# boqian333/E2ENet-Medical

Hardware: AMD Instinct MI355X
Metric: voxels/sec (train step fwd+bwd+update), 128^3 patch 32ch density=0.2 (higher is better)
Workload: dtype f32 (fp16x2 split products, f32 accumulate); 1 GPU; BraTS-shaped 4-modal 128^3 patches, shiftConvPP base 32, K=4, DSFF density 0.2, batch 2 per GPU, fwd+loss+bwd+clip+SGD+mask step, dense (parity) wgrad; parallelism=dp1

## Files before the change

### e2enet_medical_amd/_lib.py

```python
import ctypes as C
import os

_HERE = os.path.dirname(os.path.abspath(__file__))
LIB_PATH = os.environ.get("E2E_LIB_PATH") or os.path.join(_HERE, "csrc", "libe2e_hip.so")

KNOWN_ENV = frozenset({
    "E2E_CONV_MM", "E2E_MM_GRID", "E2E_MM_GEOM", "E2E_MM_PAIRQ", "E2E_CONV_DENSE", "E2E_CONV_SPARSE2", "E2E_CONV_PERSIST", "E2E_CONV_WGS",
    "E2E_CONV_KSPLIT", "E2E_WG_H2", "E2E_WG_BF3", "E2E_CT_BF3", "E2E_CT_H2",
    "E2E_CONV_DBG", "E2E_MM_STAMPS",
    "E2E_LIB_PATH", "E2E_STRICT_ENV", "E2E_DENSE_MIN_DENSITY", "E2E_MM_MIN_DENSITY", "E2E_WGRAD_STREAM", "E2E_LANES", "E2E_GRAPHS",
    "E2E_GRAPH_MAX_VOXELS", "E2E_PLAN_CACHE_GB", "E2E_SW_BLOCKING", "E2E_FORCE_DIST",
    "E2E_CPU_THREADS", "E2E_BENCH_DRY", "E2E_BENCH_DRY_FAIL_RANK", "E2E_BENCH_ALL_LAUNCHES",
})


def check_env(environ=None, strict=None):
    environ = os.environ if environ is None else environ
    unknown = sorted(k for k in environ if k.startswith("E2E_") and k not in KNOWN_ENV)
    if not unknown:
        return
    msg = ("unknown E2E_* environment variable(s) %s: not read by this build (known: %s)"
           % (", ".join(unknown), ", ".join(sorted(KNOWN_ENV))))
    if strict is None:
        strict = environ.get("E2E_STRICT_ENV") == "1"
# ... 70 lines not shown
    "e2e_conv133_sparse_eligible": (I, [I, I, I, I, I, I, I, I]),
    "e2e_conv133_sparse_wpk_floats": (LL, [I, I, I]),
    "e2e_conv133_sparse_plan": (I, [P, I, I, I, P, P, P, P, P, P]),
    "e2e_conv133_sparse_pack": (I, [P, I, LL, P]),
    "e2e_conv133_fwd_sparse": (I, [P, I, P, P, P, P, I, P, I, P, P, I, I, I, I, I, P]),
    "e2e_conv133_dgrad_sparse": (I, [P, P, P, P, I, P, P, P, I, I, I, I, I, I, I, P]),
    "e2e_conv133_fwd_dense": (I, [P, I, P, P, P, P, P, I, I, I, I, I, P, LL, P]),
    "e2e_conv133_mm_ws_bytes": (LL, [I, I, I, I, I, I, I, I, I]),
    "e2e_conv133_mm_pack": (I, [P, I, LL, P]),
    "e2e_conv133_input_ranges_ws_bytes": (LL, [I]),
    "e2e_conv133_input_ranges": (I, [P, I, P, P]),
    "e2e_absmax_word": (I, [P, LL, P, P]),
    "e2e_conv133_fwd_mm": (I, [P, I, P, P, P, P, P, P, I, I, I, I, I, P]),
    "e2e_conv133_dgrad_mm": (I, [P, P, P, P, P, I, I, I, I, I, I, P]),
    "e2e_conv133_dgrad_dense": (I, [P, P, P, P, I, I, I, I, I, I, P, LL, P]),
    "e2e_conv133_wgrad_ws_bytes": (LL, [I, I, I, I, I, I, I, I, I]),
    "e2e_conv133_wgrad": (I, [P, P, P, P, I, I, I, I, I, I, I, I, I, P, P, P]),
    "e2e_diag_split_gemm": (I, [P, P, P, I, I, P, P]),
    "e2e_diag_kernel_clock": (I, [I, P, P, I]),
    "e2e_in_stats_finalize": (I, [P, I, P, P, F, P, P, P, P, I, I, P]),
    "e2e_in_lrelu_bwd_ws_doubles": (LL, [I, I]),
    "e2e_in_lrelu_bwd": (I, [P, P, P, P, P, P, P, F, P, P, P, P, I, I, LL, P, I, P, P]),
    "e2e_convT_fwd": (I, [P, P, P, F, P, P, P, I, I, I, I, I, I, I, I, I, P, P, P]),
    "e2e_convT_dgrad": (I, [P, P, P, P, I, I, I, I, I, I, I, I, I, I, P, P, P, P]),
    "e2e_convT_wgrad_ws_bytes": (LL, [I, I, I, I, I, I, I, I, I]),
    "e2e_convT_wgrad": (I, [P, P, P, F, P, P, P, I, I, I, I, I, I, I, I, I, P, P, P, P]),
    "e2e_maxpool_fwd": (I, [P, P, P, F, P, I, I, I, I, I, I, I, I, P]),
    "e2e_maxpool_bwd_num_records": (I, [I, I, I, I, I, I]),
    "e2e_maxpool_bwd": (I, [P, P, P, F, P, P, I, I, I, I, I, I, I, I, I, P, P, P, P]),
    "e2e_head1x1_fwd": (I, [P, P, P, F, P, P, I, I, I, LL, P]),
    "e2e_head1x1_dgrad": (I, [P, P, P, I, I, I, I, LL, P]),
    "e2e_head1x1_wgrad_ws_bytes": (LL, [I, I, I, LL]),
    "e2e_head1x1_wgrad": (I, [P, P, P, F, P, P, P, I, I, I, LL, P]),
    "e2e_loss_ws_bytes": (LL, [I, I]),
    "e2e_dc_ce_reduce": (I, [P, P, P, I, I, LL, P]),
    "e2e_dc_ce_grad": (I, [P, P, P, F, I, F, P, P, I, I, LL, P]),
    "e2e_dc_ce_fold_batch": (I, [P, I, I, P]),
    "e2e_online_eval_counts": (I, [P, P, P, I, I, LL, P]),
    "e2e_dc_bce_reduce": (I, [P, P, P, P, I, I, LL, P]),
    "e2e_dc_bce_grad": (I, [P, P, P, P, F, I, F, P, P, I, I, LL, P]),
    "e2e_online_eval_regions": (I, [P, P, P, P, I, I, LL, P]),
    "e2e_seg_to_regions": (I, [P, P, P, I, I, LL, P]),
    "e2e_ds_target_gather": (I, [P, P, P, P, P, I, I, I, I, I, I, I, P]),
    "e2e_grad_sqnorm": (I, [P, I, P, P]),
    "e2e_sgd_clip_mask_step": (I, [P, I, P, F, F, F, F, I, I, P]),
    "e2e_apply_mask": (I, [P, I, P]),
    "e2e_dsff_kernel_l1": (I, [P, P, I, I, I, I, I, P]),
    "e2e_dsff_kth_value": (I, [P, I, I, P, P, P]),
    "e2e_dsff_death": (I, [P, P, P, I, P]),
    "e2e_dsff_grad_score": (I, [P, P, F, P, P, I, I, I, I, I, P]),
    "e2e_dsff_grow_above": (I, [P, P, P, I, I, I, P]),
    "e2e_dsff_expand": (I, [P, P, P, P, I, I, I, P]),
    "e2e_dsff_expand_quads": (I, [P, P, P, I, I, P]),
    "e2e_dsff_kmask_from_weights": (I, [P, P, I, I, I, P]),
    "e2e_flip3d": (I, [P, P, I, I, I, I, I, P]),
    "e2e_softmax_flip_acc": (I, [P, P, F, I, I, I, I, I, I, P]),
    "e2e_nonlin_flip_acc": (I, [P, P, F, I, I, I, I, I, I, I, P]),
    "e2e_sw_accumulate": (I, [P, P, P, P, I, I, I, I, I, I, I, I, I, I, P]),
    "e2e_sw_finalize_argmax": (I, [P, P, P, P, I, I, I, I, I, I, I, I, I, I, P]),
    "e2e_ensemble_accumulate": (I, [P, P, LL, I, I, P]),
    "e2e_export_argmax_u8": (I, [P, P, I, LL, I, I, I, LL, LL, LL, I, I, I, I, I, I, P, I, P]),
    "e2e_resample_linear": (I, [P, P, I, LL, I, I, I, LL, LL, LL, I, I, I, I, P]),
    "e2e_softmax_to_f16": (I, [P, P, I, LL, I, I, I, LL, LL, LL, P]),
    "e2e_merge_softmax_f16": (I, [P, I, I, I, I, I, P, I, I, I, I, I, I, P, I, P, P]),
    "e2e_aug_spatial": (I, [P, P, P, P, P, P, P, I, I, I, I, I, I, I, I, I, I, F, P]),
    "e2e_aug_bspline_prefilter_axis": (I, [P, P, I, I, I, I, I, P]),
# ... 26 lines not shown
    "e2e_pp_crop": (I, [P, P, P, P, P, I, I, I, I, I, I, I, I, I, I, I, F, P]),
    "e2e_pp_label_hist_bins": (I, []),
    "e2e_pp_label_hist": (I, [P, LL, P, I, P]),
    "e2e_pp_nan_to_zero": (I, [P, LL, P]),
    "e2e_pp_minmax_ws_bytes": (LL, [I, I, I, I, I]),
    "e2e_pp_minmax": (I, [P, P, P, I, LL, I, I, I, LL, LL, LL, I, P]),
    "e2e_pp_pad_edge": (I, [P, P, I, LL, I, I, I, LL, LL, LL, I, I, I, P]),
    "e2e_pp_resize_cubic": (I, [P, P, P, I, I, I, I, I, I, I, I, I, P]),
    "e2e_pp_resize_seg": (I, [P, P, I, LL, I, I, I, LL, LL, LL, I, I, I, I, P]),
    "e2e_pp_norm_ws_bytes": (LL, [I]),
    "e2e_pp_norm_stats": (I, [P, P, P, P, P, I, LL, P]),
    "e2e_pp_normalize": (I, [P, P, P, P, I, LL, P]),
    "e2e_pp_select_chunk": (I, []),
    "e2e_pp_select_max_classes": (I, []),
    "e2e_pp_select_ws_bytes": (LL, [LL, I]),
    "e2e_pp_select_count": (I, [P, LL, P, I, P, P, P]),
    "e2e_pp_select_coords": (I, [P, I, I, I, P, I, P, P, P, P, P, P]),
    "e2e_fingerprint_sample_chunk": (I, []),
    "e2e_fingerprint_sample_ws_bytes": (LL, [LL]),
    "e2e_fingerprint_sample_count": (I, [P, LL, P, P, P]),
    "e2e_fingerprint_sample_gather": (I, [P, P, I, LL, I, P, LL, P, P]),
    "e2e_fingerprint_stats_max_ranks": (I, []),
    "e2e_fingerprint_stats_ws_bytes": (LL, []),
    "e2e_fingerprint_stats": (I, [P, LL, P, I, P, P, P]),
    "e2e_loader_crop_max_batch": (I, []),
    "e2e_loader_crop": (I, [P, I, I, I, I, I, P, P, I, F, F, P]),
    "e2e_nifti_decode_f32": (I, [P, LL, I, I, I, C.c_double, C.c_double, P, P]),
    "e2e_nifti_decode_u8": (I, [P, LL, I, I, I, C.c_double, C.c_double, P, P, P]),
    "e2e_nifti_scan_grid_voxels": (LL, [I]),
    "e2e_nifti_scan": (I, [P, LL, I, I, I, C.c_double, C.c_double, P, P]),
}

_NO_STATUS = {"e2e_last_error", "e2e_abi_version", "e2e_last_kernel", "e2e_conv133_num_partials", "e2e_conv133_wgrad_ws_bytes", "e2e_conv133_dense_ws_bytes", "e2e_conv133_mm_ws_bytes", "e2e_conv133_sparse_eligible", "e2e_conv133_sparse_wpk_floats", "e2e_maxpool_bwd_num_records", "e2e_conv133_fwd_ws_bytes", "e2e_conv133_dgrad_ws_bytes",
              "e2e_convT_wgrad_ws_bytes", "e2e_conv133_input_ranges_ws_bytes", "e2e_in_lrelu_bwd_ws_doubles", "e2e_head1x1_wgrad_ws_bytes", "e2e_loss_ws_bytes", "e2e_aug_stats_ws_bytes",
              "e2e_surface_max_line", "e2e_surface_distances_ws_bytes", "e2e_cc_ws_bytes", "e2e_ct_ws_bytes", "e2e_pp_nonzero_ws_bytes", "e2e_pp_label_hist_bins",
              "e2e_pp_minmax_ws_bytes", "e2e_pp_norm_ws_bytes", "e2e_pp_select_chunk", "e2e_pp_select_max_classes", "e2e_pp_select_ws_bytes",
              "e2e_fingerprint_sample_chunk", "e2e_fingerprint_sample_ws_bytes", "e2e_fingerprint_stats_max_ranks",
              "e2e_fingerprint_stats_ws_bytes", "e2e_eval_census_max_slots", "e2e_eval_census_chunk", "e2e_eval_census_workgroups",
              "e2e_loader_crop_max_batch", "e2e_nifti_scan_grid_voxels"}


class E2EError(RuntimeError):
    pass


class _Lib:
    def __init__(self, path):
        if not os.path.exists(path):
            raise ImportError(
                "libe2e_hip.so not found at %s: build it with `python -c 'import __graft_entry__ as g; g.build()'` "
                "or `make -C e2enet_medical_amd/csrc`. There is no CPU fallback." % path)
        self._dll = C.CDLL(path)
        self.path = path
        for name, (res, args) in SIGNATURES.items():
            fn = getattr(self._dll, name)
            fn.restype = res
            fn.argtypes = args
            if name in _NO_STATUS:
                setattr(self, name[4:], fn)
            else:
                setattr(self, name[4:], self._checked(name, fn))

    def _checked(self, name, fn):
        last_error = self._dll.e2e_last_error

        def call(*a):
            rc = fn(*a)
            if rc != 0:
                raise E2EError("%s failed (%d): %s" % (name, rc, (last_error() or b"").decode()))
        call.__name__ = name
        return call


_lib = None


ABI_VERSION = 27


def lib() -> _Lib:
    global _lib
    if _lib is None:
        import torch
        check_env()
        handle = _Lib(LIB_PATH)
        got = handle.abi_version()
        if got != ABI_VERSION:
            raise ImportError("%s reports ABI version %d, this package needs %d: rebuild with `make -C %s`"
                              % (LIB_PATH, got, ABI_VERSION, os.path.dirname(LIB_PATH)))
        _lib = handle
    return _lib
```

### e2enet_medical_amd/csrc/api.hip

```cpp
#include "e2e_common.h"
#include <cstring>

namespace e2e {
static thread_local char g_err[512] = "";
void set_error(const char* fmt, ...) {
  va_list ap;
  va_start(ap, fmt);
  vsnprintf(g_err, sizeof(g_err), fmt, ap);
  va_end(ap);
}
static thread_local char g_kernel[160] = "";
void note_kernel(const char* fmt, ...) {
  va_list ap;
  va_start(ap, fmt);
  vsnprintf(g_kernel, sizeof(g_kernel), fmt, ap);
  va_end(ap);
}
}

extern "C" const char* e2e_last_error(void) { return e2e::g_err; }
extern "C" const char* e2e_last_kernel(void) { return e2e::g_kernel; }
extern "C" int e2e_abi_version(void) { return 27; }

extern "C" int e2e_diag_kernel_clock(int family, double* mhz, double* busy_ms, int reset) {
  E2E_REQUIRE(mhz != nullptr && (family == 0 || family == 1), "diag_kernel_clock: family 0 (conv133_mm) or 1 (conv133_wgrad v5)");
  if (hipDeviceSynchronize() != hipSuccess) return e2e::check_launch("diag_kernel_clock");
  unsigned long long v[2] = {0, 0};
  if (family == 0) e2e::mm_clock_read(v, reset != 0); else e2e::wgrad_clock_read(v, reset != 0);
  *mhz = v[1] ? 100.0 * (double)v[0] / (double)v[1] : 0.0;
  if (busy_ms) *busy_ms = (double)v[1] / 1e5;
  return e2e::check_launch("diag_kernel_clock");
}
```

### e2enet_medical_amd/csrc/pool_head.hip

```cpp
#include "e2e_common.h"

namespace {

__global__ __launch_bounds__(256) void maxpool_fwd_kernel(const float* __restrict__ x, const float* __restrict__ scale,
                                                          const float* __restrict__ shift, float slope,
                                                          float* __restrict__ y, int D, int H, int W, int kd, int kh, int kw,
                                                          int Do, int Ho, int Wo) {
  const int nc = blockIdx.y;
  const long long ospatial = (long long)Do * Ho * Wo;
  const long long oi = (long long)blockIdx.x * 256 + threadIdx.x;
  if (oi >= ospatial) return;
  const int wo = (int)(oi % Wo);
  const long long r = oi / Wo;
  const int ho = (int)(r % Ho), dq = (int)(r / Ho);
  float a = 1.f, b = 0.f, sl = 1.f;
  if (scale) { a = scale[nc]; b = shift[nc]; sl = slope; }
  const float* xp = x + (long long)nc * D * H * W;
  float m = -INFINITY;
  for (int i = 0; i < kd; ++i)
    for (int j = 0; j < kh; ++j)
      for (int k = 0; k < kw; ++k) {
        const float v = e2e::in_act(xp[((long long)(dq * kd + i) * H + (ho * kh + j)) * W + (wo * kw + k)], a, b, sl);
        m = (v > m || v != v) ? v : m;
      }
// ... 359 lines not shown
          const float z[4] = {e2e::in_act(q.x, a[i], b[i], sl[i]), e2e::in_act(q.y, a[i], b[i], sl[i]),
                              e2e::in_act(q.z, a[i], b[i], sl[i]), e2e::in_act(q.w, a[i], b[i], sl[i])};
#pragma unroll
          for (int k = 0; k < KB; ++k)
#pragma unroll
            for (int j = 0; j < 4; ++j) acc[i][k] = fmaf(g[k][j], z[j], acc[i][k]);
        }
      }
    }
    const int wave = threadIdx.x >> 6, lane = threadIdx.x & 63;
#pragma unroll
    for (int i = 0; i < CG; ++i)
#pragma unroll
      for (int k = 0; k < KB; ++k) {
        const double t = e2e::wave_sum_d((double)acc[i][k]);
        if (lane == 0) sh[wave][i * KB + k] = t;
      }
    __syncthreads();
    if (threadIdx.x < CG * KB) {
      const int i = threadIdx.x / KB, k = threadIdx.x - i * KB;
      if (c0 + i < C && k0 + k < K)
        atomicAdd(&acc_out[(long long)(k0 + k) * C + c0 + i],
                  sh[0][threadIdx.x] + sh[1][threadIdx.x] + sh[2][threadIdx.x] + sh[3][threadIdx.x]);
    }
    __syncthreads();
  }
}

__global__ void d2f_kernel(const double* __restrict__ src, float* __restrict__ dst, long long n) {
  const long long i = (long long)blockIdx.x * blockDim.x + threadIdx.x;
  if (i < n) dst[i] = (float)src[i];
}

}

extern "C" int e2e_maxpool_fwd(const float* x, const float* scale, const float* shift, float slope, float* y, int B,
                               int C, int D, int H, int W, int kd, int kh, int kw, void* stream) {
  E2E_REQUIRE(x && y, "maxpool_fwd: null pointer");
  E2E_REQUIRE(kd >= 1 && kh >= 1 && kw >= 1 && D >= kd && H >= kh && W >= kw, "maxpool_fwd: bad dims");
  const int Do = D / kd, Ho = H / kh, Wo = W / kw;
  if (kw == 2 && (W % 4) == 0) {
    dim3 grid2((unsigned)e2e::cdivll((long long)Do * Ho * (Wo / 2), 256), B * C);
    hipLaunchKernelGGL(maxpool_fwd_w2_kernel, grid2, dim3(256), 0, (hipStream_t)stream, x, scale, shift, slope, y, D, H, W, kd,
                       kh, Do, Ho, Wo);
    return e2e::check_launch("maxpool_fwd_w2_kernel");
  }
  dim3 grid((unsigned)e2e::cdivll((long long)Do * Ho * Wo, 256), B * C);
  hipLaunchKernelGGL(maxpool_fwd_kernel, grid, dim3(256), 0, (hipStream_t)stream, x, scale, shift, slope, y, D, H, W, kd, kh,
                     kw, Do, Ho, Wo);
  return e2e::check_launch("maxpool_fwd_kernel");
}

extern "C" int e2e_maxpool_bwd_num_records(int D, int H, int W, int kd, int kh, int kw) {
  if (kd < 1 || kh < 1 || kd > 2 || kh > 2 || kw != 2 || (W % 4) != 0 || D % kd || H % kh) return 0;
  return (int)e2e::cdivll((long long)(D / kd) * (H / kh) * (W / 4), 256);
}

extern "C" int e2e_maxpool_bwd(const float* x, const float* scale, const float* shift, float slope, const float* dy,
                               float* dx, int accumulate, int B, int C, int D, int H, int W, int kd, int kh, int kw,
                               const float* mean, const float* rstd, double* tile_sums, void* stream) {
  E2E_REQUIRE(x && dy && dx, "maxpool_bwd: null pointer");
  E2E_REQUIRE(kd >= 1 && kh >= 1 && kw >= 1 && D >= kd && H >= kh && W >= kw, "maxpool_bwd: bad dims");
  E2E_REQUIRE(tile_sums == nullptr || (mean && rstd && scale && e2e_maxpool_bwd_num_records(D, H, W, kd, kh, kw) > 0),
              "maxpool_bwd: fused InstanceNorm-backward sums need a normalised source and a shape of e2e_maxpool_bwd_num_records");
  hipStream_t st = (hipStream_t)stream;
  const int Do = D / kd, Ho = H / kh, Wo = W / kw;
// ... 48 lines not shown
  return e2e::check_launch("head_dgrad_kernel");
}

extern "C" long long e2e_head1x1_wgrad_ws_bytes(int B, int C, int K, long long spatial) {
  (void)B; (void)spatial;
  return (long long)C * K * (long long)sizeof(double);
}

extern "C" int e2e_head1x1_wgrad(const float* x, const float* scale, const float* shift, float slope,
                                 const float* dlogits, float* dw, void* ws, int B, int C, int K, long long spatial,
                                 void* stream) {
  E2E_REQUIRE(x && dlogits && dw && ws, "head1x1_wgrad: null pointer");
  hipStream_t st = (hipStream_t)stream;
  double* acc = reinterpret_cast<double*>(ws);
  e2e::zero_async(acc, (size_t)C * K * sizeof(double), st);
  long long blocks = e2e::cdivll(spatial, 256 * 16);
  if (blocks > 128) blocks = 128;
  if (blocks < 1) blocks = 1;
  if (spatial % 4 == 0 && K <= 16) {
    long long b4 = e2e::cdivll(spatial, 1024 * 8);
    if (b4 > 256) b4 = 256;
    if (b4 < 1) b4 = 1;
    dim3 grid4((unsigned)b4, e2e::cdiv(C, 8));
    if (K <= 4) hipLaunchKernelGGL((head_wgrad_v4_kernel<4, 8>), grid4, dim3(256), 0, st, x, scale, shift, slope, dlogits, acc, C, K, spatial, B);
    else hipLaunchKernelGGL((head_wgrad_v4_kernel<8, 8>), grid4, dim3(256), 0, st, x, scale, shift, slope, dlogits, acc, C, K, spatial, B);
  } else {
  dim3 grid((unsigned)blocks, C);
  DISPATCH_KB(K, hipLaunchKernelGGL((head_wgrad_kernel<KB>), grid, dim3(256), 0, st, x, scale, shift, slope, dlogits, acc, C, K,
                                    spatial, B));
  }
  hipLaunchKernelGGL(d2f_kernel, dim3((unsigned)e2e::cdivll((long long)C * K, 256)), dim3(256), 0, st, acc, dw, (long long)C * K);
  return e2e::check_launch("head1x1_wgrad");
}
```

### e2enet_medical_amd/engine.py

```python
import contextlib
import ctypes as C
import math
import os
from typing import Dict, List, Optional, Sequence, Tuple

import torch

import numpy as np

from ._lib import lib, InChan, OutChan, ParamEntry, SparsePackJob, InSumChan, MmPackJob, RangeSrc, RangeJob

LRELU_SLOPE = 0.01
IN_EPS = 1e-5
DENSE_MIN_DENSITY = float(os.environ.get("E2E_DENSE_MIN_DENSITY", "0.5"))
WGRAD_STREAM = os.environ.get("E2E_WGRAD_STREAM", "1") != "0"
WGRAD_STREAM_MAX_ELEMS = 40000000
WGRAD_LATE = True
LANES = os.environ.get("E2E_LANES", "1") != "0"
LANE_DIVS = None


def _lane_divs(voxels):
    if LANE_DIVS is not None:
        return LANE_DIVS
# ... 520 lines not shown

    def backward(self):
        s = self.src
        b, c, d, h, w = s.shape
        fuse = FUSE_IN_SUMS >= 1 and s.normed and s.last_writer is self and s.producer is not None and s.producer.own_sums is not None
        lib().maxpool_bwd(s.data.data_ptr(), _ptr(s.scale), _ptr(s.shift), LRELU_SLOPE, self.out.grad.data_ptr(),
                          s.grad.data_ptr(), self.acc, b, c, d, h, w, *self.kernel,
                          s.mean.data_ptr() if fuse else None, s.rstd.data_ptr() if fuse else None,
                          s.producer.own_sums.data_ptr() if fuse else None, _stream())
        if fuse:
            s.sums_ready = True


class HeadOp:

    def __init__(self, eng, w_name, src: Act, num_classes):
        self.eng, self.w_name, self.src, self.k = eng, w_name, src, num_classes
        b, c = src.shape[:2]
        self.out = Act(w_name, (b, num_classes) + src.shape[2:], False, eng.device)
        self.acc = 0
        self.active = True

    def plan_backward(self):
        self.src.alloc_grad()
        self.acc = self.src.claim_grad_write(self)

    def forward(self):
        s = self.src
        b, c = s.shape[:2]
        lib().head1x1_fwd(s.data.data_ptr(), _ptr(s.scale), _ptr(s.shift), LRELU_SLOPE,
                          self.eng.params[self.w_name].data_ptr(), self.out.data.data_ptr(), b, c, self.k, s.spatial,
                          _stream())

    def backward(self):
        s, e = self.src, self.eng
        b, c = s.shape[:2]
        L = lib()
        with _wgrad_stream(e, s.data.numel()) as ws:
            L.head1x1_wgrad(s.data.data_ptr(), _ptr(s.scale), _ptr(s.shift), LRELU_SLOPE, self.out.grad.data_ptr(),
                            e.grads[self.w_name].data_ptr(), ws.data_ptr(), b, c, self.k, s.spatial, _stream())
        L.head1x1_dgrad(self.out.grad.data_ptr(), e.params[self.w_name].data_ptr(), s.grad.data_ptr(), self.acc, b, c,
                        self.k, s.spatial, _stream())


class NetConfig:

    def __init__(self, in_channels, base_features, num_classes, pool_kernels, convs_per_stage=2, max_features=320,
                 shift_size=5, graph="unetpp"):
        if graph not in ("unetpp", "unet"):
            raise ValueError("graph must be 'unetpp' (unetpp_d.py) or 'unet' (unetpp_d_nodff.py)")
        self.graph = graph
        if graph == "unetpp" and len(pool_kernels) != 5:
            raise ValueError("shiftConvPP needs exactly 5 pooling stages, got %d" % len(pool_kernels))
        self.in_channels, self.base_features, self.num_classes = in_channels, base_features, num_classes
        self.pool_kernels = [tuple(int(v) for v in k) for k in pool_kernels]
        self.convs_per_stage, self.max_features = convs_per_stage, max_features
        if shift_size < 1 or shift_size % 2 == 0:
            raise ValueError("shift_size must be odd and >= 1 (reference unetpp_d.py:89 uses 5; 1 disables the shift)")
        self.shift_size = shift_size
        feats, f = [], base_features
        for _ in range(len(pool_kernels) + 1):
            feats.append(min(f, max_features))
            f = min(int(round(f * 2)), max_features)
        self.feats = feats

    @property
    def num_pool(self):
        return len(self.pool_kernels)

    def nest_nodes(self, z):
# ... 71 lines not shown

    def _build_unetpp(self, cfg):
        P = cfg.num_pool
        nodes = {}
        cur = self.input
        for st in range(P + 1):
            stride = (1, 1, 1) if st == 0 else cfg.pool_kernels[st - 1]
            for bi, prefix in enumerate(cfg.encoder_prefixes(st)):
                op = self._add_conv(prefix, [cur], cfg.feats[st], stride if bi == 0 else (1, 1, 1))
                cur = op.out
            nodes[(st, 0)] = cur
            if st == 0:
                continue
            z = P - st
            for m, lvl in cfg.nest_nodes(z):
                j = st - lvl
                up = UpOp(self, "up%d.%d.weight" % (z, m), nodes[(lvl + 1, j - 1)], cfg.feats[lvl], cfg.pool_kernels[lvl])
                self.ops.append(up)
                self.up_ops[up.w_name] = up
                srcs = [nodes[(lvl, j - 1)], up.out]
                if lvl > 0:
                    pool = PoolOp(self, "down%d.%d" % (z, m), nodes[(lvl - 1, j - 1)], cfg.pool_kernels[lvl - 1])
                    self.ops.append(pool)
                    srcs.append(pool.out)
                t = None
                for prefix in cfg.loc_prefixes(z, m):
                    op = self._add_conv(prefix, srcs if t is None else [t], cfg.feats[lvl], (1, 1, 1))
                    t = op.out
                nodes[(lvl, j)] = t
        self.nodes = nodes
        for h in range(4):
            head = HeadOp(self, "seg_outputs.%d.weight" % h, nodes[(h, P - h)], cfg.num_classes)
            self.heads.append(head)
            self.ops.append(head)

    def _build_unet(self, cfg):
        P = cfg.num_pool
        skips, cur = [], self.input
        for st in range(P + 1):
            stride = (1, 1, 1) if st == 0 else cfg.pool_kernels[st - 1]
            for bi, prefix in enumerate(cfg.encoder_prefixes(st)):
                op = self._add_conv(prefix, [cur], cfg.feats[st], stride if bi == 0 else (1, 1, 1))
                cur = op.out
            if st < P:
                skips.append(cur)
        self.nodes = {(st, 0): a for st, a in enumerate(skips)}
        by_u = []
        for u in range(P):
            lvl = P - 1 - u
            up = UpOp(self, "tu.%d.weight" % u, cur, cfg.feats[lvl], cfg.pool_kernels[lvl])
            self.ops.append(up)
            self.up_ops[up.w_name] = up
            t = None
            for prefix in cfg.unet_loc_prefixes(u):
                op = self._add_conv(prefix, [up.out, skips[lvl]] if t is None else [t], cfg.feats[lvl], (1, 1, 1))
                t = op.out
            cur = t
            self.nodes[(lvl, 1)] = t
            head = HeadOp(self, "seg_outputs.%d.weight" % u, t, cfg.num_classes)
            self.ops.append(head)
            by_u.append(head)
        self.heads = [by_u[-1]] + by_u[:-1][::-1]

    def _add_conv(self, prefix, sources, cout, stride):
        op = ConvOp(self, prefix, sources, cout, stride)
        self.ops.append(op)
        self.conv_ops[op.w_name] = op
        return op

    def set_kernel_masks(self, kmasks: Dict[str, torch.Tensor]):
        L = lib()
        self.maps_generation += 1
        self._graphs.clear()
        self._graph_seen.clear()
        self._sparse_jobs = None
        for name, op in list(self.conv_ops.items()) + list(self.up_ops.items()):
            km = kmasks.get(name)
            if isinstance(op, ConvOp):
                op.build_sparse_plans(km)
            if km is None:
                op.live = op.live_t = None
                op.density = 1.0
                continue
            r, cc = km.shape
            op.density = float(km.float().mean().item())
            km = km.to(device=self.device, dtype=torch.uint8).contiguous()
            if isinstance(op, ConvOp):
                rows = torch.empty(((r + 3) // 4) * ((cc + 7) // 8), dtype=torch.int32, device=self.device)
                cols = torch.empty(((cc + 3) // 4) * ((r + 7) // 8), dtype=torch.int32, device=self.device)
                L.dsff_expand_quads(km.data_ptr(), rows.data_ptr(), cols.data_ptr(), r, cc, _stream())
                op.live, op.live_t = rows, cols
            else:
                rows = torch.empty(r * ((cc + 31) // 32), dtype=torch.int32, device=self.device)
                cols = torch.empty(cc * ((r + 31) // 32), dtype=torch.int32, device=self.device)
                L.dsff_expand(km.data_ptr(), None, rows.data_ptr(), cols.data_ptr(), r, cc, 1, _stream())
# ... 222 lines not shown
        if self._backward_ready:
            return
        for op in (self.ops[i] for i in self._bwd_order):
            op.out.alloc_grad()
            op.plan_backward()
        order, seen = [], set()
        for op in (self.ops[i] for i in self._bwd_order):
            if isinstance(op, ConvOp):
                produced = [op.w_name, op.prefix + ".conv.bias", op.prefix + ".instnorm.weight", op.prefix + ".instnorm.bias"]
            elif isinstance(op, (UpOp, HeadOp)):
                produced = [op.w_name]
            else:
                produced = []
            for name in produced:
                if name in self.params and name not in seen:
                    order.append((name, op))
                    seen.add(name)
        order += [(name, None) for name in self.params if name not in seen]
        offs, total = {}, 0
        for name, _ in order:
            offs[name] = total
            total += (self.params[name].numel() + 63) // 64 * 64
        self.grad_flat = torch.zeros(total, dtype=torch.float32, device=self.device)
        for name, p in self.params.items():
            self.grads[name] = self.grad_flat[offs[name]:offs[name] + p.numel()].view(p.shape)
        self._bucket_after_op, lo, nb = {}, 0, 4
        for i, (name, op) in enumerate(order):
            end = offs[name] + (self.params[name].numel() + 63) // 64 * 64
            last_of_op = i + 1 == len(order) or order[i + 1][1] is not op
            if op is not None and last_of_op and (end - lo >= total // nb):
                self._bucket_after_op[id(op)] = (lo, end)
                lo = end
        self._bucket_tail = (lo, total)
        ws = max([op.wgrad_ws_bytes() for op in self.ops if hasattr(op, "wgrad_ws_bytes")] +
                 [lib().head1x1_wgrad_ws_bytes(self.batch, h.src.shape[1], h.k, h.src.spatial) for h in self.heads])
        self._wgrad_ws = [torch.empty((ws + 3) // 4, dtype=torch.float32, device=self.device) for _ in range(len(self.lane_divs) + 1)]
        cmax = max(op.cout for op in self.conv_ops.values())
        self._in_sums = [torch.zeros(int(lib().in_lrelu_bwd_ws_doubles(self.batch, cmax)), dtype=torch.float64, device=self.device)
                         for _ in range(len(self.lane_divs) + 1)]
        for op in self.conv_ops.values():
            d_, h_, w_ = op.out_dims
            lw = op.out.last_writer
            op.own_sums, op.own_np = None, 0
            if isinstance(lw, PoolOp) and FUSE_IN_SUMS >= 1:
                op.own_np = int(lib().maxpool_bwd_num_records(d_, h_, w_, *lw.kernel))
            elif isinstance(lw, ConvOp) and FUSE_IN_SUMS >= 2 and lw.sparse_ok:
                op.own_np = d_ * ((h_ + 15) // 16) * ((w_ + 31) // 32)
            if op.own_np > 0:
                op.own_sums = torch.zeros(self.batch * op.cout * op.own_np * 2, dtype=torch.float64, device=self.device)
            if op.sp_bwd is not None:
                op.sp_bwd.table = None
        self._plan_lanes_backward()
        self._loss_buffers()
        self._backward_ready = True

    def backward(self, dlogits: Optional[Sequence[Optional[torch.Tensor]]] = None):
        self.prepare_backward()
        if dlogits is not None:
            for h, g in zip(self.heads, dlogits):
                if g is None:
                    h.out.grad.zero_()
                else:
                    h.out.grad.copy_(g)
        for op in self.conv_ops.values():
            op.out.sums_ready = False
        self._refresh_weight_caches("b")
        hook = self.grad_bucket_hook
        main = torch.cuda.current_stream()
        if WGRAD_STREAM and not self._graph_ok() and not torch.cuda.is_current_stream_capturing():
            if self._wg_side is None:
                self._wg_side = torch.cuda.Stream(device=self.device)
                self.wgrad_ws_side = torch.empty_like(self._wgrad_ws[0])
            self._wg_active = self._wg_side
        side = self._wg_active

        def act(op):
            if isinstance(op, HeadOp) and not op.active:
                if op.acc == 0:
# ... 135 lines not shown
```

### include/e2e_hip.h

```cpp
#ifndef E2E_HIP_H
#define E2E_HIP_H

#ifdef __cplusplus
extern "C" {
#endif

#define E2E_OK 0
#define E2E_ERR_ARG (-1)
#define E2E_ERR_LAUNCH (-2)
#define E2E_ERR_UNSUPPORTED (-3)

const char* e2e_last_error(void);
int e2e_abi_version(void);
const char* e2e_last_kernel(void);

typedef struct {
  const float* ptr;
  const float* scale;
  const float* shift;
  long long nstride;
  int ab_nstride;
  int dshift;
  float slope;
  int reserved;
// ... 110 lines not shown
                          float* scale, float* shift, float* mean, float* rstd, int B, int C, void* stream);

long long e2e_in_lrelu_bwd_ws_doubles(int B, int C);
int e2e_in_lrelu_bwd(float* dz_dy, const float* y, const float* mean, const float* rstd, const float* scale, const float* shift,
                     const float* gamma, float slope, float* dgamma, float* dbeta, float* dbias, float* sums,
                     int B, int C, long long spatial, const double* tile_sums, int np, unsigned* dy_absmax, void* stream);

int e2e_convT_fwd(const float* x, const float* scale, const float* shift, float slope, const float* w,
                  const unsigned* live, float* y, int B, int Cin, int Cout, int D, int H, int W, int kd,
                  int kh, int kw, const unsigned* x_absmax, const unsigned* w_absmax, void* stream);
int e2e_convT_dgrad(const float* dy, const float* w, const unsigned* live_t, float* dx, int accumulate, int B,
                    int Cin, int Cout, int D, int H, int W, int kd, int kh, int kw, const unsigned* w_absmax,
                    const unsigned* dy_bound_a, const unsigned* dy_bound_b, void* stream);
long long e2e_convT_wgrad_ws_bytes(int B, int Cin, int Cout, int D, int H, int W, int kd, int kh, int kw);
int e2e_convT_wgrad(const float* x, const float* scale, const float* shift, float slope, const float* dy,
                    float* dw, void* ws, int B, int Cin, int Cout, int D, int H, int W, int kd, int kh, int kw,
                    const unsigned* x_absmax, const unsigned* dy_bound_a, const unsigned* dy_bound_b, void* stream);

int e2e_maxpool_fwd(const float* x, const float* scale, const float* shift, float slope, float* y, int B, int C,
                    int D, int H, int W, int kd, int kh, int kw, void* stream);
int e2e_maxpool_bwd_num_records(int D, int H, int W, int kd, int kh, int kw);
int e2e_maxpool_bwd(const float* x, const float* scale, const float* shift, float slope, const float* dy,
                    float* dx, int accumulate, int B, int C, int D, int H, int W, int kd, int kh, int kw,
                    const float* mean, const float* rstd, double* tile_sums, void* stream);

int e2e_head1x1_fwd(const float* x, const float* scale, const float* shift, float slope, const float* w,
                    float* logits, int B, int C, int K, long long spatial, void* stream);
int e2e_head1x1_dgrad(const float* dlogits, const float* w, float* dx, int accumulate, int B, int C, int K,
                      long long spatial, void* stream);
long long e2e_head1x1_wgrad_ws_bytes(int B, int C, int K, long long spatial);
int e2e_head1x1_wgrad(const float* x, const float* scale, const float* shift, float slope,
                      const float* dlogits, float* dw, void* ws, int B, int C, int K, long long spatial,
                      void* stream);

long long e2e_loss_ws_bytes(int B, int K);
int e2e_dc_ce_reduce(const float* logits, const float* target, void* acc, int B, int K, long long spatial,
                     void* stream);
int e2e_dc_ce_grad(const float* logits, const float* target, const void* acc, float weight, int batch_dice,
                   float smooth, float* dlogits, float* loss_out, int B, int K, long long spatial, void* stream);
int e2e_dc_ce_fold_batch(void* acc, int B, int K, void* stream);
int e2e_online_eval_counts(const float* logits, const float* target, long long* counts, int B, int K,
                           long long spatial, void* stream);

int e2e_dc_bce_reduce(const float* logits, const float* target, const unsigned* region_words, void* acc, int B, int R,
                      long long spatial, void* stream);
int e2e_dc_bce_grad(const float* logits, const float* target, const unsigned* region_words, const void* acc, float weight,
                    int batch_dice, float smooth, float* dlogits, float* loss_out, int B, int R, long long spatial,
                    void* stream);
int e2e_online_eval_regions(const float* logits, const float* target, const unsigned* region_words, long long* counts, int B,
                            int R, long long spatial, void* stream);
int e2e_seg_to_regions(const float* seg, const unsigned* region_words, float* out, int B, int R, long long spatial,
                       void* stream);

int e2e_ds_target_gather(const float* seg, float* out, const int* idx_d, const int* idx_h, const int* idx_w,
                         int BC, int D, int H, int W, int d, int h, int w, void* stream);


typedef struct {
  float* param;
  const float* grad;
  float* momentum;
  const float* mask;
  long long numel;
} e2e_param_t;
int e2e_grad_sqnorm(const e2e_param_t* table, int n, double* sq_out , void* stream);
int e2e_sgd_clip_mask_step(const e2e_param_t* table, int n, const double* sq_norm, float max_norm, float lr,
// ... 151 lines not shown
```

Baseline: 129.8 million voxels/s.

## Fuse head 1x1 wgrad, dgrad and InstanceNorm-backward sums into one pass

Adds a single-pass head backward kernel that reads dlogits and the normalised source once, producing dx, per-chunk wgrad partials and the InstanceNorm-backward sums together, followed by a small reduction kernel for dw. The aim is to remove the separate wgrad, dgrad and later IN-sum passes over the full-resolution head inputs. Heads are also moved to run right after their producer so the sums can be fused. The cost is a double-precision partial buffer sized by chunks, plus a changed op order.

```diff
diff --git a/e2enet_medical_amd/_lib.py b/e2enet_medical_amd/_lib.py
--- a/e2enet_medical_amd/_lib.py
+++ b/e2enet_medical_amd/_lib.py
@@ -126,6 +126,9 @@
     "e2e_head1x1_dgrad": (I, [P, P, P, I, I, I, I, LL, P]),
     "e2e_head1x1_wgrad_ws_bytes": (LL, [I, I, I, LL]),
     "e2e_head1x1_wgrad": (I, [P, P, P, F, P, P, P, I, I, I, LL, P]),
+    "e2e_head1x1_bwd_num_records": (I, [LL]),
+    "e2e_head1x1_bwd_ws_bytes": (LL, [I, I, I, LL]),
+    "e2e_head1x1_bwd": (I, [P, P, P, F, P, P, P, I, P, P, P, P, P, I, I, I, LL, P]),
     "e2e_loss_ws_bytes": (LL, [I, I]),
     "e2e_dc_ce_reduce": (I, [P, P, P, I, I, LL, P]),
     "e2e_dc_ce_grad": (I, [P, P, P, F, I, F, P, P, I, I, LL, P]),
@@ -218,7 +221,7 @@
 }
 
 _NO_STATUS = {"e2e_last_error", "e2e_abi_version", "e2e_last_kernel", "e2e_conv133_num_partials", "e2e_conv133_wgrad_ws_bytes", "e2e_conv133_dense_ws_bytes", "e2e_conv133_mm_ws_bytes", "e2e_conv133_sparse_eligible", "e2e_conv133_sparse_wpk_floats", "e2e_maxpool_bwd_num_records", "e2e_conv133_fwd_ws_bytes", "e2e_conv133_dgrad_ws_bytes",
-              "e2e_convT_wgrad_ws_bytes", "e2e_conv133_input_ranges_ws_bytes", "e2e_in_lrelu_bwd_ws_doubles", "e2e_head1x1_wgrad_ws_bytes", "e2e_loss_ws_bytes", "e2e_aug_stats_ws_bytes",
+              "e2e_convT_wgrad_ws_bytes", "e2e_conv133_input_ranges_ws_bytes", "e2e_in_lrelu_bwd_ws_doubles", "e2e_head1x1_wgrad_ws_bytes", "e2e_head1x1_bwd_num_records", "e2e_head1x1_bwd_ws_bytes", "e2e_loss_ws_bytes", "e2e_aug_stats_ws_bytes",
               "e2e_surface_max_line", "e2e_surface_distances_ws_bytes", "e2e_cc_ws_bytes", "e2e_ct_ws_bytes", "e2e_pp_nonzero_ws_bytes", "e2e_pp_label_hist_bins",
               "e2e_pp_minmax_ws_bytes", "e2e_pp_norm_ws_bytes", "e2e_pp_select_chunk", "e2e_pp_select_max_classes", "e2e_pp_select_ws_bytes",
               "e2e_fingerprint_sample_chunk", "e2e_fingerprint_sample_ws_bytes", "e2e_fingerprint_stats_max_ranks",
@@ -261,7 +264,7 @@
 _lib = None
 
 
-ABI_VERSION = 27
+ABI_VERSION = 28
 
 
 def lib() -> _Lib:
diff --git a/e2enet_medical_amd/csrc/api.hip b/e2enet_medical_amd/csrc/api.hip
--- a/e2enet_medical_amd/csrc/api.hip
+++ b/e2enet_medical_amd/csrc/api.hip
@@ -20,7 +20,7 @@
 
 extern "C" const char* e2e_last_error(void) { return e2e::g_err; }
 extern "C" const char* e2e_last_kernel(void) { return e2e::g_kernel; }
-extern "C" int e2e_abi_version(void) { return 27; }
+extern "C" int e2e_abi_version(void) { return 28; }
 
 extern "C" int e2e_diag_kernel_clock(int family, double* mhz, double* busy_ms, int reset) {
   E2E_REQUIRE(mhz != nullptr && (family == 0 || family == 1), "diag_kernel_clock: family 0 (conv133_mm) or 1 (conv133_wgrad v5)");
diff --git a/e2enet_medical_amd/csrc/pool_head.hip b/e2enet_medical_amd/csrc/pool_head.hip
--- a/e2enet_medical_amd/csrc/pool_head.hip
+++ b/e2enet_medical_amd/csrc/pool_head.hip
@@ -415,6 +415,121 @@
   if (i < n) dst[i] = (float)src[i];
 }
 
+constexpr int HEAD_BWD_CHUNK = 4096;
+constexpr int HEAD_BWD_CB = 32;
+constexpr int HEAD_BWD_MIN_WGS = 512;
+
+template <int KB, int VG>
+__global__ __launch_bounds__(256) void head_bwd_v4_kernel(const float* __restrict__ x, const float* __restrict__ scale,
+                                                          const float* __restrict__ shift, float slope,
+                                                          const float* __restrict__ dl, const float* __restrict__ w,
+                                                          float* __restrict__ dx, int accumulate,
+                                                          const float* __restrict__ mean, const float* __restrict__ rstd,
+                                                          double* __restrict__ sums, double* __restrict__ wrec, int C, int K,
+                                                          long long spatial, int cpb) {
+  constexpr int Q = KB + 2;
+  const int n = blockIdx.y, chunk = blockIdx.x, nchunks = gridDim.x;
+  const int wave = threadIdx.x >> 6, lane = threadIdx.x & 63;
+  __shared__ double sh[4][HEAD_BWD_CB][Q];
+  const long long base = (long long)chunk * HEAD_BWD_CHUNK;
+  const int cb = blockIdx.z * cpb;
+  const int ce = C - cb < cpb ? C - cb : cpb;
+  for (int pass = 0; pass < 4 / VG; ++pass) {
+    float g[VG][KB][4];
+    long long v[VG];
+#pragma unroll
+    for (int i = 0; i < VG; ++i) {
+      v[i] = base + ((long long)(pass * VG + i) * 256 + threadIdx.x) * 4;
+#pragma unroll
+      for (int k = 0; k < KB; ++k) {
+        float4 q = make_float4(0.f, 0.f, 0.f, 0.f);
+        if (k < K && v[i] < spatial) q = *reinterpret_cast<const float4*>(dl + ((long long)n * K + k) * spatial + v[i]);
+        g[i][k][0] = q.x; g[i][k][1] = q.y; g[i][k][2] = q.z; g[i][k][3] = q.w;
+      }
+    }
+    for (int ci = 0; ci < ce; ++ci) {
+      const int c = cb + ci;
+      const long long nc = (long long)n * C + c;
+      float a = 1.f, b = 0.f, sl = 1.f, mu = 0.f, rs = 0.f;
+      if (scale) { a = scale[nc]; b = shift[nc]; sl = slope; }
+      if (sums != nullptr) { mu = mean[nc]; rs = rstd[nc]; }
+      float wk[KB];
+#pragma unroll
+      for (int k = 0; k < KB; ++k) wk[k] = k < K ? w[(long long)k * C + c] : 0.f;
+      float4 q[VG], old[VG];
+#pragma unroll
+      for (int i = 0; i < VG; ++i) {
+        q[i] = make_float4(0.f, 0.f, 0.f, 0.f);
+        old[i] = make_float4(0.f, 0.f, 0.f, 0.f);
+        if (v[i] < spatial) {
+          q[i] = *reinterpret_cast<const float4*>(x + nc * spatial + v[i]);
+          if (accumulate) old[i] = *reinterpret_cast<const float4*>(dx + nc * spatial + v[i]);
+        }
+      }
+      float wa[KB], s1 = 0.f, s2 = 0.f;
+#pragma unroll
+      for (int k = 0; k < KB; ++k) wa[k] = 0.f;
+#pragma unroll
+      for (int i = 0; i < VG; ++i) {
+        if (v[i] >= spatial) continue;
+        const float ys[4] = {q[i].x, q[i].y, q[i].z, q[i].w};
+        const float ov[4] = {old[i].x, old[i].y, old[i].z, old[i].w};
+        float dz[4];
+#pragma unroll
+        for (int j = 0; j < 4; ++j) {
+          const float u = fmaf(ys[j], a, b);
+          const float z = u > 0.f ? u : u * sl;
+#pragma unroll
+          for (int k = 0; k < KB; ++k) wa[k] = fmaf(g[i][k][j], z, wa[k]);
+          float s = 0.f;
+#pragma unroll
+          for (int k = 0; k < KB; ++k)
+            if (k < K) s = fmaf(wk[k], g[i][k][j], s);
+          if (accumulate) s += ov[j];
+          dz[j] = s;
+          const float du = u > 0.f ? s : s * sl;
+          s1 += du;
+          s2 = fmaf(du, (ys[j] - mu) * rs, s2);
+        }
+        *reinterpret_cast<float4*>(dx + nc * spatial + v[i]) = make_float4(dz[0], dz[1], dz[2], dz[3]);
+      }
+#pragma unroll
+      for (int k = 0; k < KB; ++k) {
+        if (k >= K) continue;
+        const double t = e2e::wave_sum_dpp_d((double)wa[k]);
+        if (lane == 0) sh[wave][ci][k] = pass == 0 ? t : sh[wave][ci][k] + t;
+      }
+      if (sums != nullptr) {
+        const double t1 = e2e::wave_sum_dpp_d((double)s1), t2 = e2e::wave_sum_dpp_d((double)s2);
+        if (lane == 0) {
+          sh[wave][ci][KB] = pass == 0 ? t1 : sh[wave][ci][KB] + t1;
+          sh[wave][ci][KB + 1] = pass == 0 ? t2 : sh[wave][ci][KB + 1] + t2;
+        }
+      }
+    }
+  }
+  __syncthreads();
+  for (int idx = threadIdx.x; idx < ce * Q; idx += 256) {
+    const int ci = idx / Q, qi = idx - ci * Q, c = cb + ci;
+    if (qi < KB ? qi >= K : sums == nullptr) continue;
+    const double t = sh[0][ci][qi] + sh[1][ci][qi] + sh[2][ci][qi] + sh[3][ci][qi];
+    if (qi < KB) wrec[((long long)n * nchunks + chunk) * K * C + (long long)qi * C + c] = t;
+    else sums[(((long long)n * C + c) * nchunks + chunk) * 2 + (qi - KB)] = t;
+  }
+}
+
+__global__ __launch_bounds__(256) void head_wrec_sum_kernel(const double* __restrict__ wrec, float* __restrict__ dw, int nrec,
+                                                            int KC) {
+  const int i = blockIdx.x;
+  double a = 0.0;
+  for (int r = threadIdx.x; r < nrec; r += 256) a += wrec[(long long)r * KC + i];
+  a = e2e::wave_sum_d(a);
+  __shared__ double sh[4];
+  if ((threadIdx.x & 63) == 0) sh[threadIdx.x >> 6] = a;
+  __syncthreads();
+  if (threadIdx.x == 0) dw[i] = (float)(sh[0] + sh[1] + sh[2] + sh[3]);
+}
+
 }
 
 extern "C" int e2e_maxpool_fwd(const float* x, const float* scale, const float* shift, float slope, float* y, int B,
@@ -529,3 +644,50 @@
   hipLaunchKernelGGL(d2f_kernel, dim3((unsigned)e2e::cdivll((long long)C * K, 256)), dim3(256), 0, st, acc, dw, (long long)C * K);
   return e2e::check_launch("head1x1_wgrad");
 }
+
+extern "C" int e2e_head1x1_bwd_num_records(long long spatial) {
+  if (spatial <= 0 || spatial % 4 != 0) return 0;
+  return (int)e2e::cdivll(spatial, HEAD_BWD_CHUNK);
+}
+
+static bool head_bwd_fused(int K, long long spatial) { return K <= 16 && e2e_head1x1_bwd_num_records(spatial) > 0; }
+
+extern "C" long long e2e_head1x1_bwd_ws_bytes(int B, int C, int K, long long spatial) {
+  if (!head_bwd_fused(K, spatial)) return e2e_head1x1_wgrad_ws_bytes(B, C, K, spatial);
+  return (long long)B * e2e_head1x1_bwd_num_records(spatial) * C * K * (long long)sizeof(double);
+}
+
+extern "C" int e2e_head1x1_bwd(const float* x, const float* scale, const float* shift, float slope, const float* dlogits,
+                               const float* w, float* dx, int accumulate, float* dw, void* ws, const float* mean,
+                               const float* rstd, double* sums, int B, int C, int K, long long spatial, void* stream) {
+  E2E_REQUIRE(x && dlogits && w && dx && dw && ws, "head1x1_bwd: null pointer");
+  E2E_REQUIRE(B > 0 && C > 0 && K > 0 && spatial > 0, "head1x1_bwd: bad dims");
+  if (!head_bwd_fused(K, spatial)) {
+    E2E_REQUIRE(sums == nullptr, "head1x1_bwd: fused InstanceNorm-backward sums need a shape of e2e_head1x1_bwd_num_records and K <= 16");
+    int rc = e2e_head1x1_wgrad(x, scale, shift, slope, dlogits, dw, ws, B, C, K, spatial, stream);
+    if (rc != E2E_OK) return rc;
+    rc = e2e_head1x1_dgrad(dlogits, w, dx, accumulate, B, C, K, spatial, stream);
+    if (rc == E2E_OK) e2e::note_kernel("head_wgrad_kernel+d2f_kernel+head_dgrad_kernel");
+    return rc;
+  }
+  E2E_REQUIRE(sums == nullptr || (mean && rstd && scale), "head1x1_bwd: fused InstanceNorm-backward sums need a normalised source");
+  hipStream_t st = (hipStream_t)stream;
+  const int nrec = e2e_head1x1_bwd_num_records(spatial);
+  double* wrec = reinterpret_cast<double*>(ws);
+  int cpb = HEAD_BWD_CB;
+  while (cpb > 1 && (long long)nrec * B * e2e::cdiv(C, cpb) < HEAD_BWD_MIN_WGS) cpb >>= 1;
+  dim3 grid((unsigned)nrec, B, e2e::cdiv(C, cpb));
+  if (K <= 4)
+    hipLaunchKernelGGL((head_bwd_v4_kernel<4, 4>), grid, dim3(256), 0, st, x, scale, shift, slope, dlogits, w, dx, accumulate, mean,
+                       rstd, sums, wrec, C, K, spatial, cpb);
+  else if (K <= 8)
+    hipLaunchKernelGGL((head_bwd_v4_kernel<8, 2>), grid, dim3(256), 0, st, x, scale, shift, slope, dlogits, w, dx, accumulate, mean,
+                       rstd, sums, wrec, C, K, spatial, cpb);
+  else
+    hipLaunchKernelGGL((head_bwd_v4_kernel<16, 1>), grid, dim3(256), 0, st, x, scale, shift, slope, dlogits, w, dx, accumulate, mean,
+                       rstd, sums, wrec, C, K, spatial, cpb);
+  hipLaunchKernelGGL(head_wrec_sum_kernel, dim3(C * K), dim3(256), 0, st, (const double*)wrec, dw, B * nrec, C * K);
+  e2e::note_kernel("head_bwd_v4_kernel<%d> wgs=%d cpb=%d sums=%d", K <= 4 ? 4 : K <= 8 ? 8 : 16, nrec * B * e2e::cdiv(C, cpb), cpb,
+                   sums != nullptr ? 1 : 0);
+  return e2e::check_launch("head_bwd_v4_kernel");
+}
diff --git a/e2enet_medical_amd/engine.py b/e2enet_medical_amd/engine.py
--- a/e2enet_medical_amd/engine.py
+++ b/e2enet_medical_amd/engine.py
@@ -576,10 +576,29 @@
                           self.eng.params[self.w_name].data_ptr(), self.out.data.data_ptr(), b, c, self.k, s.spatial,
                           _stream())
 
+    @property
+    def one_pass(self):
+        return self.k <= 16 and lib().head1x1_bwd_num_records(self.src.spatial) > 0
+
+    def wgrad_ws_bytes(self):
+        b, c = self.src.shape[:2]
+        return max(lib().head1x1_wgrad_ws_bytes(b, c, self.k, self.src.spatial),
+                   lib().head1x1_bwd_ws_bytes(b, c, self.k, self.src.spatial))
+
     def backward(self):
         s, e = self.src, self.eng
         b, c = s.shape[:2]
         L = lib()
+        if self.one_pass:
+            fuse = (FUSE_IN_SUMS >= 1 and s.normed and s.last_writer is self and s.producer is not None
+                    and s.producer.own_sums is not None)
+            L.head1x1_bwd(s.data.data_ptr(), _ptr(s.scale), _ptr(s.shift), LRELU_SLOPE, self.out.grad.data_ptr(),
+                          e.params[self.w_name].data_ptr(), s.grad.data_ptr(), self.acc, e.grads[self.w_name].data_ptr(),
+                          e.wgrad_ws.data_ptr(), s.mean.data_ptr() if fuse else None, s.rstd.data_ptr() if fuse else None,
+                          s.producer.own_sums.data_ptr() if fuse else None, b, c, self.k, s.spatial, _stream())
+            if fuse:
+                s.sums_ready = True
+            return
         with _wgrad_stream(e, s.data.numel()) as ws:
             L.head1x1_wgrad(s.data.data_ptr(), _ptr(s.scale), _ptr(s.shift), LRELU_SLOPE, self.out.grad.data_ptr(),
                             e.grads[self.w_name].data_ptr(), ws.data_ptr(), b, c, self.k, s.spatial, _stream())
@@ -717,7 +736,7 @@
         for h in range(4):
             head = HeadOp(self, "seg_outputs.%d.weight" % h, nodes[(h, P - h)], cfg.num_classes)
             self.heads.append(head)
-            self.ops.append(head)
+            self._place_head(head)
 
     def _build_unet(self, cfg):
         P = cfg.num_pool
@@ -746,6 +765,14 @@
             self.ops.append(head)
             by_u.append(head)
         self.heads = [by_u[-1]] + by_u[:-1][::-1]
+
+    def _place_head(self, head):
+        src = head.src
+        writers = 1 + sum(1 for op in self.ops for a in self._reads(op) if a is src)
+        if src.producer is None or src.producer not in self.ops or writers > 2:
+            self.ops.append(head)
+        else:
+            self.ops.insert(self.ops.index(src.producer) + 1, head)
 
     def _add_conv(self, prefix, sources, cout, stride):
         op = ConvOp(self, prefix, sources, cout, stride)
@@ -1034,8 +1061,7 @@
                 self._bucket_after_op[id(op)] = (lo, end)
                 lo = end
         self._bucket_tail = (lo, total)
-        ws = max([op.wgrad_ws_bytes() for op in self.ops if hasattr(op, "wgrad_ws_bytes")] +
-                 [lib().head1x1_wgrad_ws_bytes(self.batch, h.src.shape[1], h.k, h.src.spatial) for h in self.heads])
+        ws = max(op.wgrad_ws_bytes() for op in self.ops if hasattr(op, "wgrad_ws_bytes"))
         self._wgrad_ws = [torch.empty((ws + 3) // 4, dtype=torch.float32, device=self.device) for _ in range(len(self.lane_divs) + 1)]
         cmax = max(op.cout for op in self.conv_ops.values())
         self._in_sums = [torch.zeros(int(lib().in_lrelu_bwd_ws_doubles(self.batch, cmax)), dtype=torch.float64, device=self.device)
@@ -1046,6 +1072,8 @@
             op.own_sums, op.own_np = None, 0
             if isinstance(lw, PoolOp) and FUSE_IN_SUMS >= 1:
                 op.own_np = int(lib().maxpool_bwd_num_records(d_, h_, w_, *lw.kernel))
+            elif isinstance(lw, HeadOp) and FUSE_IN_SUMS >= 1 and lw.one_pass:
+                op.own_np = int(lib().head1x1_bwd_num_records(op.out.spatial))
             elif isinstance(lw, ConvOp) and FUSE_IN_SUMS >= 2 and lw.sparse_ok:
                 op.own_np = d_ * ((h_ + 15) // 16) * ((w_ + 31) // 32)
             if op.own_np > 0:
diff --git a/include/e2e_hip.h b/include/e2e_hip.h
--- a/include/e2e_hip.h
+++ b/include/e2e_hip.h
@@ -166,6 +166,11 @@
 int e2e_head1x1_wgrad(const float* x, const float* scale, const float* shift, float slope,
                       const float* dlogits, float* dw, void* ws, int B, int C, int K, long long spatial,
                       void* stream);
+int e2e_head1x1_bwd_num_records(long long spatial);
+long long e2e_head1x1_bwd_ws_bytes(int B, int C, int K, long long spatial);
+int e2e_head1x1_bwd(const float* x, const float* scale, const float* shift, float slope, const float* dlogits,
+                    const float* w, float* dx, int accumulate, float* dw, void* ws, const float* mean,
+                    const float* rstd, double* sums, int B, int C, int K, long long spatial, void* stream);
 
 long long e2e_loss_ws_bytes(int B, int K);
 int e2e_dc_ce_reduce(const float* logits, const float* target, void* acc, int B, int K, long long spatial,
```

Result: faster. 131.2 million voxels/s, median of 6 (+1.1%).
